# davide-coccomini/MINTIME-Multi-Identity-size-iNvariant-TIMEsformer-for-Video-Deepfake-Detection

Measured on AMD Instinct MI355X. Metric: clips/sec (8-frame, 2-identity, 224^2 crops) fwd+bwd, higher is better.
Workload: dtype f32; 1 GPU; config 3: EfficientNet-B0 + SizeInvariantTimeSformer(dim 512, depth 9, heads 8), B=32/GPU, 8 frames, 2 identities (identity-masked), 224x224 crops, random-init seeded weights (restored before every step), train-mode BN + drop-connect 0.2, step = fwd + BCE loss + bwd + SGD(lr .01, wd 1e-4); global_batch=32, frames=8, parallelism=dp1

## Files before the change

mintime-multi-identity-size-invariant-timesformer-for-video-deepfake-detection_amd/csrc/gemm_planes.hip:

```cpp
#include "../../include/mintime_hip.h"
#include "common.hpp"
#include "gemm_planes_launch.hpp"
#include "gemm_geometry.hpp"
#include "det.hpp"
#include <string.h>

using namespace mt;

namespace {

__device__ __forceinline__ void to_blk_block(const float* __restrict__ src, int64_t ld, int R, int C, const PlaneRef& o, int rb, int cb, int lane) {
  const int r = rb * 32 + (lane >> 1), c = cb * 16 + (lane & 1) * 8;
  float x[8] = {0.f, 0.f, 0.f, 0.f, 0.f, 0.f, 0.f, 0.f};
  if (r < R) {
    const float* s = src + (int64_t)r * ld + c;
    if (c + 8 <= C && ((ld & 3) == 0) && (((uintptr_t)src & 15) == 0)) {
      const float4 u = *reinterpret_cast<const float4*>(s), v = *reinterpret_cast<const float4*>(s + 4);
      x[0] = u.x; x[1] = u.y; x[2] = u.z; x[3] = u.w; x[4] = v.x; x[5] = v.y; x[6] = v.z; x[7] = v.w;
    } else {
#pragma unroll
      for (int e = 0; e < 8; ++e) if (c + e < C) x[e] = s[e];
    }
  }
  planes_store8(o, r, c, x);
}

__global__ __launch_bounds__(256) void split_planes_blk_kernel(const float* __restrict__ src, int64_t ld, int R, int C, PlaneRef o) {
  const int wave = threadIdx.x >> 6, lane = threadIdx.x & 63;
  const int rb = blockIdx.y, cb = blockIdx.x * 4 + wave;
  if (cb >= o.cb16) return;
  to_blk_block(src, ld, R, C, o, rb, cb, lane);
}

__global__ __launch_bounds__(256) void bn_bwd_apply_planes_kernel(const float* __restrict__ du, const float* __restrict__ z,
                                                                  const float* __restrict__ kabc, int R, int C, PlaneRef o) {
  const int wave = threadIdx.x >> 6, lane = threadIdx.x & 63;
  const int rb = blockIdx.y, cb = blockIdx.x * 4 + wave;
  if (cb >= o.cb16) return;
  const int r = rb * 32 + (lane >> 1), c = cb * 16 + (lane & 1) * 8;
  float x[8] = {0.f, 0.f, 0.f, 0.f, 0.f, 0.f, 0.f, 0.f};
  if (r < R) {
#pragma unroll
    for (int e = 0; e < 8; e += 4) {
      if (c + e + 4 <= C) {
        const float4 a = *reinterpret_cast<const float4*>(du + (int64_t)r * C + c + e), b = *reinterpret_cast<const float4*>(z + (int64_t)r * C + c + e);
        const float4 ka = *reinterpret_cast<const float4*>(kabc + c + e), kb = *reinterpret_cast<const float4*>(kabc + C + c + e),
                     kc = *reinterpret_cast<const float4*>(kabc + 2 * C + c + e);
        x[e] = fmaf(ka.x, a.x, fmaf(kb.x, b.x, kc.x)); x[e + 1] = fmaf(ka.y, a.y, fmaf(kb.y, b.y, kc.y));
        x[e + 2] = fmaf(ka.z, a.z, fmaf(kb.z, b.z, kc.z)); x[e + 3] = fmaf(ka.w, a.w, fmaf(kb.w, b.w, kc.w));
      }
    }
  }
  planes_store8(o, r, c, x);
}

struct SplitItem { const float* src; __bf16* planes; int64_t rows, cols, first; };

__global__ __launch_bounds__(256) void split_planes_blk_multi_kernel(const SplitItem* __restrict__ items, int count, int64_t total) {
  const int64_t wb = (int64_t)blockIdx.x * 4 + (threadIdx.x >> 6);
  if (wb >= total) return;
  int lo = 0, hi = count - 1;
  while (lo < hi) { const int mid = (lo + hi + 1) >> 1; if (items[mid].first <= wb) lo = mid; else hi = mid - 1; }
  const SplitItem it = items[lo];
  const int R = (int)it.rows, Cc = (int)it.cols;
  const int cb16 = (Cc + 15) >> 4, rp = (R + 31) & ~31;
  const int64_t loc = wb - it.first;
  const PlaneRef o{it.planes, (int64_t)rp * cb16 * 16, cb16, rp};
  to_blk_block(it.src, Cc, R, Cc, o, (int)(loc / cb16), (int)(loc % cb16), threadIdx.x & 63);
}

constexpr int kSkMaxGrid = 1024;
constexpr int64_t kSkFlagBytes = 4096;

int cu_count() {
  static int cus[64] = {0};
  int dev = 0;
  (void)hipGetDevice(&dev);
  int& c = cus[dev & 63];
  if (c == 0) {
    hipDeviceProp_t pr;
    c = hipGetDeviceProperties(&pr, dev) == hipSuccess && pr.multiProcessorCount > 0 ? pr.multiProcessorCount : 256;
  }
  return c;
}

int g_persist = -1;
int persist_blocks() {
  if (g_persist < 0) {
    g_persist = env_int("MT_PLANES_PERSIST", 0);
    if (g_persist < 0 || g_persist > 4) g_persist = 0;
  }
  return g_persist;
}

}

extern "C" int mt_gemm_planes_set_persist(int blocks_per_cu) {
  const int prev = persist_blocks();
  g_persist = blocks_per_cu < 0 || blocks_per_cu > 4 ? 0 : blocks_per_cu;
  return prev;
}

extern "C" int64_t mt_gemm_planes_workspace_bytes(void) { return kSkFlagBytes + (int64_t)kSkMaxGrid * 128 * 128 * 4; }

extern "C" int64_t mt_planes_elems(int rows, int cols) {
  if (rows <= 0 || cols <= 0) return 0;
  return (int64_t)((rows + 31) & ~31) * ((cols + 15) & ~15);
}

extern "C" int mt_split_planes_blk(const float* src, int64_t ld, int rows, int cols, void* planes, void* stream) {
  if (!src || !planes) return fail(MT_ERR_ARG, "mt_split_planes_blk: null pointer");
  if (rows <= 0 || cols <= 0 || ld < cols) return fail(MT_ERR_ARG, "mt_split_planes_blk: bad shape %d x %d (ld %lld)", rows, cols, (long long)ld);
  if ((uintptr_t)planes & 15) return fail(MT_ERR_ARG, "mt_split_planes_blk: planes must be 16-byte aligned");
  const int cb16 = (cols + 15) >> 4, rp = (rows + 31) & ~31;
  const PlaneRef o{reinterpret_cast<__bf16*>(planes), (int64_t)rp * cb16 * 16, cb16, rp};
  hipLaunchKernelGGL(split_planes_blk_kernel, dim3((cb16 + 3) / 4, rp / 32), dim3(256), 0, (hipStream_t)stream, src, ld, rows, cols, o);
  return check_launch("mt_split_planes_blk");
}

extern "C" int mt_bn_bwd_apply_planes(const float* du, const float* z, const float* kabc, void* planes, int rows, int C, void* stream) {
  if (!du || !z || !kabc || !planes || rows <= 0 || C <= 0) return fail(MT_ERR_ARG, "mt_bn_bwd_apply_planes: bad arguments");
  if ((C & 3) || (((uintptr_t)du | (uintptr_t)z | (uintptr_t)kabc | (uintptr_t)planes) & 15))
    return fail(MT_ERR_ARG, "mt_bn_bwd_apply_planes: C %% 4 == 0 and 16-byte alignment");
  const int cb16 = (C + 15) >> 4, rp = (rows + 31) & ~31;
  const PlaneRef o{reinterpret_cast<__bf16*>(planes), (int64_t)rp * cb16 * 16, cb16, rp};
  hipLaunchKernelGGL(bn_bwd_apply_planes_kernel, dim3((cb16 + 3) / 4, rp / 32), dim3(256), 0, (hipStream_t)stream, du, z, kabc, rows, C, o);
  return check_launch("mt_bn_bwd_apply_planes");
}

extern "C" int mt_split_planes_blk_multi(const void* items, int count, int64_t total_blocks, void* stream) {
  if (!items || count <= 0 || total_blocks <= 0) return fail(MT_ERR_ARG, "mt_split_planes_blk_multi: bad arguments");
  hipLaunchKernelGGL(split_planes_blk_multi_kernel, dim3((unsigned)((total_blocks + 3) / 4)), dim3(256), 0, (hipStream_t)stream,
                     reinterpret_cast<const SplitItem*>(items), count, total_blocks);
  return check_launch("mt_split_planes_blk_multi");
}

static int gemm_planes_impl(const mt_gemm_planes_desc* d, void* stream) {
  if (!d || !d->a_planes || !d->b_planes) return fail(MT_ERR_ARG, "mt_gemm_planes: null operand planes");
  if (d->M <= 0 || d->N <= 0 || d->K <= 0) return fail(MT_ERR_ARG, "mt_gemm_planes: bad shape %d %d %d", d->M, d->N, d->K);
  if (((uintptr_t)d->a_planes & 15) || ((uintptr_t)d->b_planes & 15) || ((uintptr_t)d->c_planes & 15))
    return fail(MT_ERR_ARG, "mt_gemm_planes: planes must be 16-byte aligned");
  const int op = d->op, epi = d->epilogue;
  const bool cpl = d->c_planes != nullptr;
  if (!d->C && !cpl) return fail(MT_ERR_ARG, "mt_gemm_planes: no output");
  if (cpl && epi != MT_EPI_GEGLU && epi != MT_EPI_GEGLU_BWD) return fail(MT_ERR_UNSUPPORTED, "mt_gemm_planes: plane output only from the GEGLU pair");
  if (epi == MT_EPI_BIAS_RES && !d->R) return fail(MT_ERR_ARG, "mt_gemm_planes: BIAS_RES needs R");
  if (epi == MT_EPI_GEGLU && (d->n_half * 2 != d->N || (d->n_half & 63))) return fail(MT_ERR_ARG, "mt_gemm_planes GEGLU: N must be 2*n_half, n_half %% 64 == 0");
  if (epi == MT_EPI_GEGLU_BWD && (!d->C2 || d->n_half != d->N || (d->n_half & 31)))
    return fail(MT_ERR_ARG, "mt_gemm_planes GEGLU_BWD: needs C2, n_half == N and n_half %% 32 == 0");
  hipStream_t s = (hipStream_t)stream;
  const bool high = matmul_precision() == MT_PRECISION_HIGH;
  const int np = high ? 2 : 3;
  auto launch = [&](int skm, const GemmArgs& ga, dim3 g) {
    return high ? launch_planes_high(op, epi, cpl, skm, ga, g, s) : launch_planes_form<3>(op, epi, cpl, skm, ga, g, s);
  };

  const int a_rows = op == MT_OP_TN ? d->K : d->M, a_cols = op == MT_OP_TN ? d->M : d->K;
  const int b_rows = op == MT_OP_NT ? d->N : d->K, b_cols = op == MT_OP_NT ? d->K : d->N;
  GemmArgs a;
  memset(&a, 0, sizeof(a));
  a.C = d->C; a.M = d->M; a.N = d->N; a.K = d->K; a.ldc = d->ldc;
  a.a_planes = d->a_planes; a.a_pstride = mt_planes_elems(a_rows, a_cols); a.lda = (a_cols + 15) >> 4;
  a.b_planes = d->b_planes; a.b_pstride = mt_planes_elems(b_rows, b_cols); a.ldb = (b_cols + 15) >> 4;
  if (6 * a.a_pstride > 0xFFFFFFFFll || 6 * a.b_pstride > 0xFFFFFFFFll)
    return fail(MT_ERR_UNSUPPORTED, "mt_gemm_planes: an operand's planes span %lld bytes (> 4 GB: 32-bit DMA offsets); use mt_gemm for it (lib.planes_fit)",
                (long long)(6 * (a.a_pstride > a.b_pstride ? a.a_pstride : a.b_pstride)));
  a.bias = d->bias; a.R = d->R; a.ldr = d->ldr; a.C2 = d->C2; a.ldc2 = d->ldc2; a.n_half = d->n_half; a.col_sum = d->col_sum;
  a.hw = 1; a.stats_slots = d->stats_slots != 0 ? d->stats_slots : 1; a.stats = d->stats; a.b_hw = 1; a.e_hw = 1;
  if (epi == MT_EPI_STATS && !d->stats) return fail(MT_ERR_ARG, "mt_gemm_planes: STATS needs stats");
  if (epi == MT_EPI_GEGLU_BWD)
    if (int rc = det_gemm_colsum_setup(a.det, d->M, d->n_half, d->col_sum, s)) return rc;
  if (cpl) {
    const int c_cols = epi == MT_EPI_GEGLU ? d->n_half : 2 * d->n_half;
    a.c_planes = d->c_planes; a.c_pstride = mt_planes_elems(d->M, c_cols); a.ldcp = (c_cols + 15) >> 4;
  }

  const TileGrid tg = tile_grid(d->M, d->N, 128, 128, (int64_t)128 * d->K * 2 * np);
  const int m_tiles = tg.m_tiles, n_tiles = tg.n_tiles;
  if (op == MT_OP_TN) {
    if (epi != MT_EPI_ATOMIC) return fail(MT_ERR_UNSUPPORTED, "mt_gemm_planes TN: ATOMIC epilogue only (C pre-zeroed)");
    static const int target = env_int("MT_WGRAD_BLOCKS", 640);
    const SplitK sk = split_k_ranges(d->K, m_tiles * n_tiles, d->split_k, target, 16, K_XCD);
    a.k_chunk = sk.k_chunk; a.xcd_k = sk.xcd_k;
    if (int rc = det_gemm_setup(a.C, a.ldc, a.det_slab, d->M, d->N, sk.ranges, false, s)) return rc;
    return launch(0, a, dim3(m_tiles * n_tiles, sk.grid_y, 1));
  }
  dim3 grid(tg.grid_x, 1, 1);
  a.group_n = tg.group_n;
  static const int prio = env_int("MT_PLANES_MAIN_PRIO", 0);
  a.wave_prio = prio;
  bool sk = false;
  if (d->sk_workspace && d->sk_workspace_bytes >= mt_gemm_planes_workspace_bytes() && !((uintptr_t)d->sk_workspace & 255)) {
    int g = cu_count() * 2 / 8 * 8;
    if (g > kSkMaxGrid) g = kSkMaxGrid;
    const int64_t units = (int64_t)m_tiles * n_tiles * (((d->K + 15) / 16 + 1) / 2);
    if (g >= 8 && units >= (int64_t)g * 2 && units < (1ll << 30)) {
      sk = true;
      grid = dim3((unsigned)g, 1, 1);
      a.sk_on = 1;
      a.sk_flags = reinterpret_cast<int*>(d->sk_workspace);
      a.sk_ws = reinterpret_cast<float*>(reinterpret_cast<char*>(d->sk_workspace) + kSkFlagBytes);
    }
  }
  if (!sk && !cpl && (epi == MT_EPI_STORE || epi == MT_EPI_BIAS_RES)) {
    const int per_cu = persist_blocks();
    const int g = cu_count() * per_cu / 8 * 8;
    if (per_cu > 0 && g >= 8 && m_tiles * n_tiles > g) {
      const dim3 pg((unsigned)g, 1, 1);
      const bool nt_store = op == MT_OP_NT && epi == MT_EPI_STORE, nt_bias_res = op == MT_OP_NT && epi == MT_EPI_BIAS_RES;
      const bool nn_store = op == MT_OP_NN && epi == MT_EPI_STORE;
      if (nt_store || nt_bias_res || nn_store) return launch(2, a, pg);
    }
  }
  return launch(sk ? 1 : 0, a, grid);
}

extern "C" int mt_gemm_planes(const mt_gemm_planes_desc* d, void* stream) {
  const int rc = gemm_planes_impl(d, stream);
  if (rc) { (void)mt::det_gemm_finish(nullptr, false); return rc; }
  return mt::det_gemm_finish((hipStream_t)stream, true);
}
```

mintime-multi-identity-size-invariant-timesformer-for-video-deepfake-detection_amd/csrc/gemm_planes.hpp:

```cpp
#pragma once
#include "gemm_split.hpp"
#include "planes.hpp"

#ifndef MT_PLANES_ABLATE
#define MT_PLANES_ABLATE 0
#endif
#ifndef MT_PLANES_EPI_ABLATE
#define MT_PLANES_EPI_ABLATE 0
#endif
#ifndef MT_PLANES_PRIO
#define MT_PLANES_PRIO 0
#endif

namespace mt {

typedef short s16x4_t __attribute__((ext_vector_type(4)));
enum : int { BAL_NONE = 0, BAL_PAIR = 1, BAL_PHASE = 2 };

__device__ __forceinline__ void lds_dma16_s(const void* sbase, unsigned voff, unsigned lds_byte_addr) {
  unsigned keep;
  asm volatile("s_mov_b32 %0, m0\n\ts_mov_b32 m0, %3\n\ts_nop 0\n\tglobal_load_lds_dwordx4 %1, %2\n\ts_mov_b32 m0, %0"
               : "=&s"(keep) : "v"(voff), "s"(sbase), "s"(lds_byte_addr) : "memory");
}

__device__ __forceinline__ void planes_emit_tile(const float (&v)[16], float* wl, const PlaneRef& o, int row0, int col0, int M, int lane) {
  const int col_l = lane & 31, row_h = (lane >> 5) * 4;
#pragma unroll
  for (int r = 0; r < 16; ++r) wl[((r & 3) + 8 * (r >> 2) + row_h) * 36 + col_l] = v[r];
  asm volatile("s_waitcnt lgkmcnt(0)" ::: "memory");
#pragma unroll
  for (int pass = 0; pass < 2; ++pass) {
    const int g = pass * 64 + lane, row = g >> 2, cg = g & 3;
    const float4 lo = *reinterpret_cast<const float4*>(wl + row * 36 + cg * 8);
    const float4 hi = *reinterpret_cast<const float4*>(wl + row * 36 + cg * 8 + 4);
    const int rg = row0 + row, cgl = col0 + cg * 8;
    const bool live = rg < M;
    const float x[8] = {live ? lo.x : 0.f, live ? lo.y : 0.f, live ? lo.z : 0.f, live ? lo.w : 0.f,
                        live ? hi.x : 0.f, live ? hi.y : 0.f, live ? hi.z : 0.f, live ? hi.w : 0.f};
    if (rg < o.rows_pad && cgl < o.cb16 * 16) { if (MT_PLANES_EPI_ABLATE & 8) { if (x[0] + x[7] == 123.456f) o.p[0] = (__bf16)1.f; } else planes_store8(o, rg, cgl, x); }
  }
  asm volatile("s_waitcnt lgkmcnt(0)" ::: "memory");
}

template <int TM, int TN, int EPI>
__device__ __forceinline__ void planes_epilogue(const GemmArgs& p, f32x16 (&acc)[TM][TN], int m0, int n0, int wm, int wn, int lane, float* wl) {
  static_assert(EPI == EPI_GEGLU || EPI == EPI_GEGLU_BWD, "plane output: the GEGLU pair");
  const PlaneRef o{reinterpret_cast<__bf16*>(p.c_planes), p.c_pstride, (int)p.ldcp, (p.M + 31) & ~31};
  const int col_l = lane & 31, row_h = (lane >> 5) * 4;
  const int mw = m0 + wm * TM * 32;
  if constexpr (EPI == EPI_GEGLU) {
    const int j = (n0 >> 1) + wn * 32 + col_l;
    const bool jok = j < p.n_half;
    const float ba = (jok && p.bias) ? p.bias[j] : 0.f;
    const float bg = (jok && p.bias) ? p.bias[p.n_half + j] : 0.f;
#pragma unroll
    for (int i = 0; i < TM; ++i) {
      float hv[16];
#pragma unroll
      for (int r = 0; r < 16; ++r) {
        const int m = mw + i * 32 + row_h + (r & 3) + 8 * (r >> 2);
        const float a = acc[i][0][r] + ba, g = acc[i][1][r] + bg;
        hv[r] = a * gelu_erf(g);
        if (m < p.M && jok) {
          if (p.C2) *reinterpret_cast<float2*>(p.C2 + (int64_t)m * p.ldc2 + 2 * j) = make_float2(a, g);
          if (p.C) p.C[(int64_t)m * p.ldc + j] = hv[r];
        }
      }
      planes_emit_tile(hv, wl, o, mw + i * 32, (n0 >> 1) + wn * 32, p.M, lane);
    }
  } else {
    f32x16 dgs[TM][TN];
    float s1[TN], s2[TN];
#pragma unroll
    for (int j = 0; j < TN; ++j) {
      const int n = n0 + wn * TN * 32 + j * 32 + col_l;
      const bool nok = n < p.N;
      s1[j] = 0.f; s2[j] = 0.f;
#pragma unroll
      for (int i = 0; i < TM; ++i) {
        float2 ag[16];
#pragma unroll
        for (int r = 0; r < 16; ++r) {
          const int m = mw + i * 32 + row_h + (r & 3) + 8 * (r >> 2);
          ag[r] = ((MT_PLANES_EPI_ABLATE & 1) || !(m < p.M && nok)) ? make_float2(0.3f, 0.1f)
                                                                     : *reinterpret_cast<const float2*>(p.C2 + (int64_t)m * p.ldc2 + 2 * n);
        }
#pragma unroll
        for (int r = 0; r < 16; ++r) {
          const int m = mw + i * 32 + row_h + (r & 3) + 8 * (r >> 2);
          const float v = acc[i][j][r];
          float gl, gr;
          if (MT_PLANES_EPI_ABLATE & 2) { gl = ag[r].y; gr = ag[r].y + 1.f; } else gelu_erf_both(ag[r].y, gl, gr);
          const bool live = m < p.M && nok;
          const float da = live ? v * gl : 0.f, dg = live ? v * ag[r].x * gr : 0.f;
          acc[i][j][r] = da;
          dgs[i][j][r] = dg;
          s1[j] += da; s2[j] += dg;
        }
        __builtin_amdgcn_sched_barrier(0);
      }
    }
#pragma unroll
    for (int j = 0; j < TN; ++j) {
      const int n = n0 + wn * TN * 32 + j * 32 + col_l;
      const bool nok = n < p.N;
#pragma unroll
      for (int i = 0; i < TM; ++i) {
        float da[16], dg[16];
#pragma unroll
        for (int r = 0; r < 16; ++r) {
          da[r] = acc[i][j][r]; dg[r] = dgs[i][j][r];
          const int m = mw + i * 32 + row_h + (r & 3) + 8 * (r >> 2);
          if (p.C && m < p.M && nok) { p.C[(int64_t)m * p.ldc + n] = da[r]; p.C[(int64_t)m * p.ldc + p.n_half + n] = dg[r]; }
        }
        if (MT_PLANES_EPI_ABLATE & 4) { if (da[3] + dg[5] == 123.456f) p.col_sum[0] = 1.f; }
        else if (n0 + wn * TN * 32 + j * 32 < p.N) {
          planes_emit_tile(da, wl, o, mw + i * 32, n0 + wn * TN * 32 + j * 32, p.M, lane);
          planes_emit_tile(dg, wl, o, mw + i * 32, p.n_half + n0 + wn * TN * 32 + j * 32, p.M, lane);
        }
      }
      if (p.col_sum && !(MT_PLANES_EPI_ABLATE & 16)) {
        float t1 = s1[j], t2 = s2[j];
        t1 += __shfl_xor(t1, 32);
        t2 += __shfl_xor(t2, 32);
        if (lane < 32 && nok) {
          if (p.det.vals) {
            const int rk = mw >> 5;
            det_put(p.det, n >> 5, rk, n & 31, t1);
            det_put(p.det, (p.n_half + n) >> 5, rk, n & 31, t2);
            if (rk == 0 && (n & 31) == 0) { det_base(p.det, n >> 5, n); det_base(p.det, (p.n_half + n) >> 5, p.n_half + n); }
          } else {
            atomicAdd(p.col_sum + n, t1);
            atomicAdd(p.col_sum + p.n_half + n, t2);
          }
        }
      }
    }
  }
}

template <int BM, int BN>
__device__ __forceinline__ void sk_tile_coords(const GemmArgs& p, int t, int& mt_, int& nt_) {
  const int n_tiles = (p.N + BN - 1) / BN, m_tiles = (p.M + BM - 1) / BM;
  if (p.group_n > 0) {
    const int q = m_tiles >> 3, r = m_tiles & 7;
    int xcd = 0, base = 0;
    for (; xcd < 7; ++xcd) {
      const int cnt = (q + (xcd < r ? 1 : 0)) * n_tiles;
      if (t < base + cnt) break;
      base += cnt;
    }
    const int rows = q + (xcd < r ? 1 : 0);
    const int row0 = xcd < r ? xcd * (q + 1) : r * (q + 1) + (xcd - r) * q;
    const int idx = t - base;
    const int per_group = rows * p.group_n;
    const int g = idx / per_group;
    const int rem = idx - g * per_group;
    const int groups = (n_tiles + p.group_n - 1) / p.group_n;
    const int gw = (g == groups - 1) ? n_tiles - g * p.group_n : p.group_n;
    const int ml = rem / gw;
    mt_ = row0 + ml;
    nt_ = g * p.group_n + (rem - ml * gw);
  } else {
    mt_ = t / n_tiles;
    nt_ = t - mt_ * n_tiles;
  }
}

template <int WAVES_M, int WAVES_N, int TM, int TN, bool AKM, bool BKM, int EPI, int STAGES, int MINW, int BAL, bool CPL = false, int SKM = 0, int NP = 3>
__global__ __launch_bounds__(WAVES_M * WAVES_N * 64, MINW)
void gemm_planes_kernel(const GemmArgs p) {
  constexpr int NW = WAVES_M * WAVES_N;
  constexpr int BM = WAVES_M * TM * 32;
  constexpr int BN = WAVES_N * TN * 32;
  constexpr int BK = 16;
  constexpr int A_PLANE = BM * 32, B_PLANE = BN * 32;
  static_assert(NP == 2 || NP == 3, "two or three pieces per operand");
  constexpr int STAGE = NP * (A_PLANE + B_PLANE);
  constexpr int PPA = A_PLANE / 1024, PPB = B_PLANE / 1024;
  constexpr int PA = NP * PPA, PB = NP * PPB;
  static_assert((PA + PB) % NW == 0, "every wavefront must issue the same number of DMA pieces");
  constexpr int IPW = (PA + PB) / NW;
  static_assert(STAGES >= 2 && STAGES <= 4, "2..4 stages");
  static_assert((!AKM || BM == 128) && (!BKM || BN == 128), "k-major images are laid out for 128-column tiles");
  constexpr bool SK = SKM == 1, PS = SKM == 2;
  static_assert(!SK || !AKM, "stream-K: forward / data-gradient forms (weight gradients split K over the grid already)");
  static_assert(!PS || (!AKM && !CPL && STAGES == 2 && EPI != EPI_GEGLU && BAL != BAL_PHASE), "persistent form: NT / NN, fp32 output, ring of two");
  constexpr bool PAIR = BAL == BAL_PAIR, PHASE = BAL == BAL_PHASE;

  extern __shared__ __attribute__((aligned(16))) unsigned char smem_pl[];
  const unsigned lds_base = (unsigned)(uintptr_t)(__attribute__((address_space(3))) unsigned char*)smem_pl;

  const int tid = threadIdx.x;
  const int lane = tid & 63;
  const int wave = __builtin_amdgcn_readfirstlane(tid >> 6);
  const int wm = wave / WAVES_N;
  const int wn = wave % WAVES_N;

  const __bf16* a_base = reinterpret_cast<const __bf16*>(p.a_planes);
  const __bf16* b_base = reinterpret_cast<const __bf16*>(p.b_planes);

  int a_frag[TM], b_frag[TN];
  {
    const int kh = lane >> 5;
    const int g = lane >> 4, i16 = lane & 15;
    const int ktr = 8 * (g >> 1) + (i16 >> 2);
    const int swz = 2 * (i16 >> 2);
#pragma unroll
    for (int i = 0; i < TM; ++i) {
      if constexpr (!AKM) {
        const int row = wm * TM * 32 + i * 32 + (lane & 31);
        a_frag[i] = row * 32 + ((kh ^ ((row >> 3) & 1)) << 4);
      } else {
        const int seg = (wm * TM * 32 + i * 32) / 16 + (g & 1);
        a_frag[i] = ktr * 256 + ((seg ^ swz) * 32) + (i16 & 3) * 8;
      }
    }
#pragma unroll
    for (int j = 0; j < TN; ++j) {
      if constexpr (!BKM) {
        const int row = wn * TN * 32 + j * 32 + (lane & 31);
        b_frag[j] = row * 32 + ((kh ^ ((row >> 3) & 1)) << 4);
      } else {
        const int seg = (wn * TN * 32 + j * 32) / 16 + (g & 1);
        b_frag[j] = ktr * 256 + ((seg ^ swz) * 32) + (i16 & 3) * 8;
      }
    }
  }

  struct Frags { bf16x8_t a0[TM], a1[TM], a2[NP == 3 ? TM : 1], b0[TN], b1[TN], b2[NP == 3 ? TN : 1]; };
  typedef __attribute__((address_space(3))) s16x4_t* lds_tr_p;
  typedef __attribute__((address_space(3))) const unsigned char* lds_cp;
  auto tr_read = [&](const unsigned char* base) -> bf16x8_t {
    lds_cp a = (lds_cp)base;
    const s16x4_t lo = __builtin_amdgcn_ds_read_tr16_b64_v4i16((lds_tr_p)a);
    const s16x4_t hi = __builtin_amdgcn_ds_read_tr16_b64_v4i16((lds_tr_p)(a + 1024));
    union { s16x4_t h[2]; bf16x8_t v; } u;
    u.h[0] = lo; u.h[1] = hi;
    return u.v;
  };

  auto read_frags = [&](int slot, Frags& f) {
    const unsigned char* sa = smem_pl + slot * STAGE;
    const unsigned char* sb = sa + NP * A_PLANE;
    if (MT_PLANES_ABLATE & 4) {
#pragma unroll
      for (int e = 0; e < 8; ++e) {
#pragma unroll
        for (int i = 0; i < TM; ++i) { f.a0[i][e] = (__bf16)(float)(lane + e + i); f.a1[i][e] = (__bf16)(float)(lane - e); if constexpr (NP == 3) f.a2[i][e] = (__bf16)(float)(lane ^ e); }
#pragma unroll
        for (int j = 0; j < TN; ++j) { f.b0[j][e] = (__bf16)(float)(lane * 2 + e + j); f.b1[j][e] = (__bf16)(float)(lane + 3 * e); if constexpr (NP == 3) f.b2[j][e] = (__bf16)(float)(3 + e); }
      }
      return;
    }
#pragma unroll
    for (int i = 0; i < TM; ++i) {
      if constexpr (!AKM) {
        f.a0[i] = *reinterpret_cast<const bf16x8_t*>(sa + a_frag[i]);
        f.a1[i] = *reinterpret_cast<const bf16x8_t*>(sa + A_PLANE + a_frag[i]);
        if constexpr (NP == 3) f.a2[i] = *reinterpret_cast<const bf16x8_t*>(sa + 2 * A_PLANE + a_frag[i]);
      } else {
        f.a0[i] = tr_read(sa + a_frag[i]);
        f.a1[i] = tr_read(sa + A_PLANE + a_frag[i]);
        if constexpr (NP == 3) f.a2[i] = tr_read(sa + 2 * A_PLANE + a_frag[i]);
      }
    }
#pragma unroll
    for (int j = 0; j < TN; ++j) {
      if constexpr (!BKM) {
        f.b0[j] = *reinterpret_cast<const bf16x8_t*>(sb + b_frag[j]);
        f.b1[j] = *reinterpret_cast<const bf16x8_t*>(sb + B_PLANE + b_frag[j]);
        if constexpr (NP == 3) f.b2[j] = *reinterpret_cast<const bf16x8_t*>(sb + 2 * B_PLANE + b_frag[j]);
      } else {
        f.b0[j] = tr_read(sb + b_frag[j]);
        f.b1[j] = tr_read(sb + B_PLANE + b_frag[j]);
        if constexpr (NP == 3) f.b2[j] = tr_read(sb + 2 * B_PLANE + b_frag[j]);
      }
    }
  };

  auto negate = [&](bf16x8_t& v, unsigned mask) {
    uint4 u = *reinterpret_cast<uint4*>(&v);
    u.x ^= mask; u.y ^= mask; u.z ^= mask; u.w ^= mask;
    v = *reinterpret_cast<bf16x8_t*>(&u);
  };

  f32x16 acc[TM][TN];
  f32x16 nacc[PAIR ? TM : 1][PAIR ? TN : 1];

  auto mma = [&](Frags& f, auto odd_c, unsigned phase_mask) {
    constexpr bool ODD = PAIR && decltype(odd_c)::value;
    if (MT_PLANES_ABLATE & 16) {
      float z = 0.f;
#pragma unroll
      for (int i = 0; i < TM; ++i) { z += (float)f.a0[i][0] + (float)f.a1[i][1]; if constexpr (NP == 3) z += (float)f.a2[i][2]; }
#pragma unroll
      for (int j = 0; j < TN; ++j) { z += (float)f.b0[j][0] + (float)f.b1[j][1]; if constexpr (NP == 3) z += (float)f.b2[j][2]; }
      acc[0][0][0] += z;
      return;
    }
#define MT_TERM(X, Y)                                                                                        \
  _Pragma("unroll") for (int i = 0; i < TM; ++i) _Pragma("unroll") for (int j = 0; j < TN; ++j)                 \
      acc[i][j] = __builtin_amdgcn_mfma_f32_32x32x16_bf16(f.X[i], f.Y[j], acc[i][j], 0, 0, 0);
#define MT_NTERM(X, Y)                                                                                       \
  _Pragma("unroll") for (int i = 0; i < TM; ++i) _Pragma("unroll") for (int j = 0; j < TN; ++j)                 \
      nacc[i][j] = __builtin_amdgcn_mfma_f32_32x32x16_bf16(f.X[i], f.Y[j], nacc[i][j], 0, 0, 0);
    if constexpr (PHASE) {
#pragma unroll
      for (int i = 0; i < TM; ++i) { negate(f.a0[i], phase_mask); negate(f.a1[i], phase_mask); if constexpr (NP == 3) negate(f.a2[i], phase_mask); }
    }
    if constexpr (ODD) {
#pragma unroll
      for (int i = 0; i < TM; ++i) negate(f.a0[i], 0x80008000u);
      if constexpr (NP == 3) { MT_TERM(a2, b0) MT_TERM(a1, b1) MT_NTERM(a0, b2) }
      MT_TERM(a1, b0) MT_NTERM(a0, b1) MT_NTERM(a0, b0)
    } else {
      if constexpr (NP == 3) { MT_TERM(a2, b0) MT_TERM(a1, b1) MT_TERM(a0, b2) }
      MT_TERM(a1, b0) MT_TERM(a0, b1) MT_TERM(a0, b0)
    }
#undef MT_TERM
#undef MT_NTERM
  };
  auto flip_acc = [&]() {
#pragma unroll
    for (int i = 0; i < TM; ++i)
#pragma unroll
      for (int j = 0; j < TN; ++j)
#pragma unroll
        for (int r = 0; r < 16; ++r) acc[i][j][r] = -acc[i][j][r];
  };
#define MT_PL_BARRIER() do { if (!(MT_PLANES_ABLATE & 2)) __builtin_amdgcn_s_barrier(); } while (0)

  auto run_piece = [&](int mt_, int nt_, int k_begin, int kt_lo, int nk) {
    const int m0 = mt_ * BM, n0 = nt_ * BN;
    unsigned voff[IPW];
    bool is_a[IPW];
#pragma unroll
    for (int j = 0; j < IPW; ++j) {
      const int q = wave * IPW + j;
      is_a[j] = q < PA;
      const int qq = is_a[j] ? q : q - PA;
      const int plane = is_a[j] ? qq / PPA : qq / PPB;
      const int piece = is_a[j] ? qq % PPA : qq % PPB;
      const int64_t pstride = is_a[j] ? p.a_pstride : p.b_pstride;
      const int64_t cb16 = is_a[j] ? p.lda : p.ldb;
      const bool kmaj = is_a[j] ? AKM : BKM;
      int64_t off;
      if (!kmaj) {
        const int row = lane >> 1, slot = lane & 1;
        const int kh = slot ^ ((row >> 3) & 1);
        int g0;
        int lim;
        if (is_a[j]) { g0 = m0 + piece * 32; lim = p.M; }
        else if constexpr (EPI == EPI_GEGLU) {
          static_assert(EPI != EPI_GEGLU || TN == 2, "GEGLU wants TN == 2");
          const int w = piece >> 1, sel = piece & 1;
          g0 = sel * p.n_half + (n0 >> 1) + w * 32; lim = 2 * p.n_half;
          if ((n0 >> 1) + w * 32 >= p.n_half) g0 = 0;
        } else { g0 = n0 + piece * 32; lim = p.N; }
        if (g0 >= lim) g0 = (lim - 1) & ~31;
        off = plane * pstride + (int64_t)(g0 >> 5) * cb16 * 512 + row * 16 + kh * 8;
      } else {
        const int kl = piece * 4 + (lane >> 4), s16 = lane & 15;
        const int seg = (s16 >> 1) ^ (2 * (kl & 3)), half = s16 & 1;
        int cb = ((is_a[j] ? m0 : n0) >> 4) + seg;
        const int cbmax = (int)cb16 - 1;
        cb = cb < cbmax ? cb : cbmax;
        off = plane * pstride + (int64_t)cb * 512 + kl * 16 + half * 8;
      }
      voff[j] = (unsigned)(off * 2);
    }

    auto issue = [&](int kt, int slot) {
      if (MT_PLANES_ABLATE & 1) return;
      const int kb = k_begin + (kt_lo + kt) * BK;
      const __bf16* as = a_base + (AKM ? ((int64_t)(kb >> 5) * p.lda * 512 + (kb & 31) * 16) : (int64_t)(kb >> 4) * 512);
      const __bf16* bs = b_base + (BKM ? ((int64_t)(kb >> 5) * p.ldb * 512 + (kb & 31) * 16) : (int64_t)(kb >> 4) * 512);
      const unsigned dst = lds_base + (unsigned)(slot * STAGE);
#pragma unroll
      for (int j = 0; j < IPW; ++j)
        lds_dma16_s(is_a[j] ? as : bs, voff[j], dst + (unsigned)((wave * IPW + j) * 1024));
    };

#pragma unroll
    for (int i = 0; i < TM; ++i)
#pragma unroll
      for (int j = 0; j < TN; ++j)
#pragma unroll
        for (int r = 0; r < 16; ++r) { acc[i][j][r] = 0.f; if constexpr (PAIR) nacc[i][j][r] = 0.f; }

    const int q1 = PHASE ? nk >> 2 : nk, q2 = PHASE ? nk - (nk >> 2) : nk;

#pragma unroll
    for (int s = 0; s < STAGES - 1; ++s)
      if (s < nk) issue(s, s);
    int slot = 0;
    auto step = [&](int kt, auto odd_c) {
      const int later = min(STAGES - 2, nk - 1 - kt);
      if (later >= 2) wait_vmcnt<2 * IPW>();
      else if (later == 1) wait_vmcnt<IPW>();
      else wait_vmcnt<0>();
      MT_PL_BARRIER();
      int nslot = slot + STAGES - 1; nslot = nslot >= STAGES ? nslot - STAGES : nslot;
      if (kt + STAGES - 1 < nk) issue(kt + STAGES - 1, nslot);
      Frags f;
      read_frags(slot, f);
      unsigned mask = 0;
      if constexpr (PHASE) {
        if (kt == q1 || kt == q2) flip_acc();
        mask = (kt >= q1 && kt < q2) ? 0x80008000u : 0u;
      }
      mma(f, odd_c, mask);
      slot = slot + 1 >= STAGES ? 0 : slot + 1;
    };
    for (int kt = 0; kt < nk; kt += 2) {
      step(kt, std::false_type{});
      if (kt + 1 >= nk) break;
      step(kt + 1, std::true_type{});
    }
    if constexpr (PHASE) {
      if (q2 >= nk && q1 < nk) flip_acc();
    }
    if constexpr (PAIR) {
#pragma unroll
      for (int i = 0; i < TM; ++i)
#pragma unroll
        for (int j = 0; j < TN; ++j)
#pragma unroll
          for (int r = 0; r < 16; ++r) acc[i][j][r] -= nacc[i][j][r];
#pragma unroll
      for (int i = 0; i < TM; ++i)
#pragma unroll
        for (int j = 0; j < TN; ++j) asm volatile("" : "+v"(acc[i][j]));
    }
  };

  auto epilogue = [&](int mt_, int nt_, int split_idx = -1) {
    if (MT_PLANES_ABLATE & 8) {
      float sacc = 0.f;
#pragma unroll
      for (int i = 0; i < TM; ++i)
#pragma unroll
        for (int j = 0; j < TN; ++j)
#pragma unroll
          for (int r = 0; r < 16; ++r) sacc += acc[i][j][r];
      if (sacc == 123.456f) p.C[0] = sacc;
      return;
    }
    int m0e = mt_ * BM, n0e = nt_ * BN, lane_e = lane;
    asm volatile("" : "+s"(m0e), "+s"(n0e), "+v"(lane_e));
    if constexpr (CPL) {
      static_assert(!CPL || STAGES * STAGE >= NW * 32 * 36 * 4, "the plane epilogue's LDS patches live in the main loop's stages");
      __syncthreads();
      planes_epilogue<TM, TN, EPI>(p, acc, m0e, n0e, wm, wn, lane_e, reinterpret_cast<float*>(smem_pl) + wave * (32 * 36));
    } else {
      gemm_epilogue<TM, TN, EPI>(p, acc, m0e, n0e, wm, wn, lane_e, split_idx);
    }
  };

  if (p.wave_prio == 1) __builtin_amdgcn_s_setprio(1);
  else if (p.wave_prio == 2) __builtin_amdgcn_s_setprio(2);
  else if (p.wave_prio == 3) __builtin_amdgcn_s_setprio(3);
  if (MT_PLANES_PRIO == 1) {
    const unsigned hwid = __builtin_amdgcn_s_getreg((4 << 0) | (0 << 6) | (3 << 11));
    if (__builtin_amdgcn_readfirstlane(hwid) & 1) __builtin_amdgcn_s_setprio(1);
  } else if (MT_PLANES_PRIO == 2) {
    if ((blockIdx.x >> 8) & 1) __builtin_amdgcn_s_setprio(1);
  }

  if constexpr (PS) {
    const int Q = gridDim.x >> 3, xcd = blockIdx.x & 7, q = blockIdx.x >> 3;
    const int n_tiles = (p.N + BN - 1) / BN, m_tiles = (p.M + BM - 1) / BM;
    int base = 0, cnt;
    if (p.group_n > 0) {
      const int qq = m_tiles >> 3, rr = m_tiles & 7;
      for (int i = 0; i < xcd; ++i) base += (qq + (i < rr ? 1 : 0)) * n_tiles;
      cnt = (qq + (xcd < rr ? 1 : 0)) * n_tiles;
    } else {
      const int T = m_tiles * n_tiles, per = T >> 3, rem = T & 7;
      base = xcd * per + min(xcd, rem);
      cnt = per + (xcd < rem ? 1 : 0);
    }
    if (q >= cnt) return;
    const int nk = (p.K + BK - 1) / BK;
    bool is_a[IPW];
    int pl_[IPW], pc_[IPW];
#pragma unroll
    for (int j = 0; j < IPW; ++j) {
      const int qj = wave * IPW + j;
      is_a[j] = qj < PA;
      const int qx = is_a[j] ? qj : qj - PA;
      pl_[j] = is_a[j] ? qx / PPA : qx / PPB;
      pc_[j] = is_a[j] ? qx % PPA : qx % PPB;
    }
    auto setup = [&](int mt_, int nt_, unsigned (&voff)[IPW]) {
      const int m0 = mt_ * BM, n0 = nt_ * BN;
#pragma unroll
      for (int j = 0; j < IPW; ++j) {
        const int64_t pstride = is_a[j] ? p.a_pstride : p.b_pstride;
        const int64_t cb16 = is_a[j] ? p.lda : p.ldb;
        const bool kmaj = is_a[j] ? AKM : BKM;
        int64_t off;
        if (!kmaj) {
          const int row = lane >> 1, sl = lane & 1;
          const int kh = sl ^ ((row >> 3) & 1);
          int g0 = (is_a[j] ? m0 : n0) + pc_[j] * 32;
          const int lim = is_a[j] ? p.M : p.N;
          if (g0 >= lim) g0 = (lim - 1) & ~31;
          off = pl_[j] * pstride + (int64_t)(g0 >> 5) * cb16 * 512 + row * 16 + kh * 8;
        } else {
          const int kl = pc_[j] * 4 + (lane >> 4), s16 = lane & 15;
          const int seg = (s16 >> 1) ^ (2 * (kl & 3)), half = s16 & 1;
          int cb = ((is_a[j] ? m0 : n0) >> 4) + seg;
          const int cbmax = (int)cb16 - 1;
          cb = cb < cbmax ? cb : cbmax;
          off = pl_[j] * pstride + (int64_t)cb * 512 + kl * 16 + half * 8;
        }
        voff[j] = (unsigned)(off * 2);
      }
    };
    auto issue = [&](const unsigned (&voff)[IPW], int kt, int slot_) {
      if (MT_PLANES_ABLATE & 1) return;
      const int kb = kt * BK;
      const __bf16* as = a_base + (AKM ? ((int64_t)(kb >> 5) * p.lda * 512 + (kb & 31) * 16) : (int64_t)(kb >> 4) * 512);
      const __bf16* bs = b_base + (BKM ? ((int64_t)(kb >> 5) * p.ldb * 512 + (kb & 31) * 16) : (int64_t)(kb >> 4) * 512);
      const unsigned dst = lds_base + (unsigned)(slot_ * STAGE);
#pragma unroll
      for (int j = 0; j < IPW; ++j) lds_dma16_s(is_a[j] ? as : bs, voff[j], dst + (unsigned)((wave * IPW + j) * 1024));
    };
    int i = q, mt_, nt_;
    sk_tile_coords<BM, BN>(p, base + i, mt_, nt_);
    unsigned vc[IPW], vn[IPW];
    setup(mt_, nt_, vc);
    issue(vc, 0, 0);
    int slot = 0;
    while (true) {
      const int inext = i + Q;
      const bool has_next = inext < cnt;
      int mtn = 0, ntn = 0;
      if (has_next) {
        sk_tile_coords<BM, BN>(p, base + inext, mtn, ntn);
        setup(mtn, ntn, vn);
      }
#pragma unroll
      for (int ii = 0; ii < TM; ++ii)
#pragma unroll
        for (int jj = 0; jj < TN; ++jj)
#pragma unroll
          for (int r = 0; r < 16; ++r) { acc[ii][jj][r] = 0.f; if constexpr (PAIR) nacc[ii][jj][r] = 0.f; }
      auto step = [&](int kt, auto odd_c) {
        wait_vmcnt<0>();
        MT_PL_BARRIER();
        const int nslot = slot ^ 1;
        if (kt + 1 < nk) issue(vc, kt + 1, nslot);
        else if (has_next) issue(vn, 0, nslot);
        Frags f;
        read_frags(slot, f);
        mma(f, odd_c, 0u);
        slot = nslot;
      };
      for (int kt = 0; kt < nk; kt += 2) {
        step(kt, std::false_type{});
        if (kt + 1 >= nk) break;
        step(kt + 1, std::true_type{});
      }
      if constexpr (PAIR) {
#pragma unroll
        for (int ii = 0; ii < TM; ++ii)
#pragma unroll
          for (int jj = 0; jj < TN; ++jj)
#pragma unroll
            for (int r = 0; r < 16; ++r) acc[ii][jj][r] -= nacc[ii][jj][r];
#pragma unroll
        for (int ii = 0; ii < TM; ++ii)
#pragma unroll
          for (int jj = 0; jj < TN; ++jj) asm volatile("" : "+v"(acc[ii][jj]));
      }
      epilogue(mt_, nt_);
      if (!has_next) break;
      i = inext; mt_ = mtn; nt_ = ntn;
#pragma unroll
      for (int j = 0; j < IPW; ++j) vc[j] = vn[j];
    }
  } else if constexpr (!SK) {
    int mt_, nt_;
    int k_begin = 0, k_end = p.K;
    int split_idx = blockIdx.y;
    if (p.xcd_k) {
      const int tiles = gridDim.x, lin = blockIdx.y * gridDim.x + blockIdx.x;
      const int xcd = lin & 7, idx = lin >> 3;
      const int split = xcd + 8 * (idx / tiles), t = idx % tiles;
      const int n_tiles = (p.N + BN - 1) / BN, m_tiles = (p.M + BM - 1) / BM;
      if (m_tiles >= n_tiles) { mt_ = t / n_tiles; nt_ = t - mt_ * n_tiles; }
      else { nt_ = t / m_tiles; mt_ = t - nt_ * m_tiles; }
      k_begin = split * p.k_chunk;
      k_end = min(p.K, k_begin + p.k_chunk);
      if (k_begin >= k_end) return;
      split_idx = split;
    } else {
      if (!tile_coords<BM, BN>(p, mt_, nt_)) return;
      if (p.k_chunk > 0) {
        k_begin = blockIdx.y * p.k_chunk;
        k_end = min(p.K, k_begin + p.k_chunk);
        if (k_begin >= k_end) return;
      }
    }
    const int nk = (k_end - k_begin + BK - 1) / BK;
    if (nk <= 0) return;
    run_piece(mt_, nt_, k_begin, 0, nk);
    epilogue(mt_, nt_, split_idx);
  } else {
    const int G = gridDim.x;
    const int L = (blockIdx.x & 7) * (G >> 3) + (blockIdx.x >> 3);
    const int nkt = (p.K + BK - 1) / BK;
    const int npt = (nkt + 1) >> 1;
    const int U = ((p.N + BN - 1) / BN) * ((p.M + BM - 1) / BM) * npt;
    const int uq = U / G, ur = U % G;
    int u = L * uq + min(L, ur);
    const int u_end = u + uq + (L < ur ? 1 : 0);
    constexpr int SLAB = BM * BN;
    while (u < u_end) {
      const int t = u / npt;
      const int kt0 = 2 * (u - t * npt);
      const int ulen = min(npt - (u - t * npt), u_end - u);
      const int len = min(nkt - kt0, 2 * ulen);
      int mt_, nt_;
      sk_tile_coords<BM, BN>(p, t, mt_, nt_);
      __builtin_amdgcn_s_barrier();
      run_piece(mt_, nt_, 0, kt0, len);
      u += ulen;
      if (len != nkt) {
        int lane_s = lane, wave_s = wave;
        asm volatile("" : "+v"(lane_s), "+s"(wave_s));
        const int my_off = wave_s * (TM * TN * 1024) + lane_s * 4;
        if (kt0 != 0) {
          float* slab = p.sk_ws + (int64_t)L * SLAB + my_off;
#pragma unroll
          for (int i = 0; i < TM; ++i)
#pragma unroll
            for (int j = 0; j < TN; ++j)
#pragma unroll
              for (int q = 0; q < 4; ++q)
                *reinterpret_cast<float4*>(slab + ((i * TN + j) * 4 + q) * 256) =
                    make_float4(acc[i][j][4 * q], acc[i][j][4 * q + 1], acc[i][j][4 * q + 2], acc[i][j][4 * q + 3]);
          asm volatile("s_waitcnt vmcnt(0)" ::: "memory");
          __syncthreads();
          if (tid == 0) {
            __builtin_amdgcn_fence(__ATOMIC_RELEASE, "agent");
            asm volatile("s_waitcnt vmcnt(0)" ::: "memory");
            __hip_atomic_store(p.sk_flags + L, 1, __ATOMIC_RELAXED, __HIP_MEMORY_SCOPE_AGENT);
          }
          continue;
        }
        int covered = ulen;
        for (int lb = L + 1; covered < npt; ++lb) {
          const int span = uq + (lb < ur ? 1 : 0);
          if (tid == 0) {
            int spins = 0;
            while (__hip_atomic_load(p.sk_flags + lb, __ATOMIC_RELAXED, __HIP_MEMORY_SCOPE_AGENT) == 0) {
              __builtin_amdgcn_s_sleep(8);
              if (++spins > (1 << 24)) break;
            }
            __builtin_amdgcn_fence(__ATOMIC_ACQUIRE, "agent");
          }
          __syncthreads();
          const float* slab = p.sk_ws + (int64_t)lb * SLAB + my_off;
#pragma unroll
          for (int i = 0; i < TM; ++i)
#pragma unroll
            for (int j = 0; j < TN; ++j)
#pragma unroll
              for (int q = 0; q < 4; ++q) {
                const float4 v = *reinterpret_cast<const float4*>(slab + ((i * TN + j) * 4 + q) * 256);
                acc[i][j][4 * q] += v.x; acc[i][j][4 * q + 1] += v.y; acc[i][j][4 * q + 2] += v.z; acc[i][j][4 * q + 3] += v.w;
              }
          asm volatile("s_waitcnt vmcnt(0)" ::: "memory");
          __syncthreads();
          if (tid == 0) __hip_atomic_store(p.sk_flags + lb, 0, __ATOMIC_RELAXED, __HIP_MEMORY_SCOPE_AGENT);
          covered += min(npt - covered, span);
        }
      }
      epilogue(mt_, nt_);
    }
  }
#undef MT_PL_BARRIER
}

}
```

Baseline: 719.0 clips/s.

## Restructure GEGLU backward epilogue with buffer loads and per-column-block software pipelining

The GEGLU backward epilogue now reads the saved (a, g) pairs through a bounds-checked raw buffer resource, so out-of-range lanes get zeros without per-element predication. It also prefetches the next column block's pairs while the current block is written out. The full dgs[TM][TN] register array becomes a per-j dgj[TM] buffer and each column block is stored right after it is computed, which should lower register pressure and overlap loads with stores. The column-sum reduction moves after the loop. A new ldc2 range check keeps the 32-bit buffer offsets valid, and the ag[TM][16] prefetch array costs registers in exchange.

```diff
diff --git a/mintime-multi-identity-size-invariant-timesformer-for-video-deepfake-detection_amd/csrc/gemm_planes.hip b/mintime-multi-identity-size-invariant-timesformer-for-video-deepfake-detection_amd/csrc/gemm_planes.hip
--- a/mintime-multi-identity-size-invariant-timesformer-for-video-deepfake-detection_amd/csrc/gemm_planes.hip
+++ b/mintime-multi-identity-size-invariant-timesformer-for-video-deepfake-detection_amd/csrc/gemm_planes.hip
@@ -148,6 +148,8 @@
   if (epi == MT_EPI_GEGLU && (d->n_half * 2 != d->N || (d->n_half & 63))) return fail(MT_ERR_ARG, "mt_gemm_planes GEGLU: N must be 2*n_half, n_half %% 64 == 0");
   if (epi == MT_EPI_GEGLU_BWD && (!d->C2 || d->n_half != d->N || (d->n_half & 31)))
     return fail(MT_ERR_ARG, "mt_gemm_planes GEGLU_BWD: needs C2, n_half == N and n_half %% 32 == 0");
+  if (epi == MT_EPI_GEGLU_BWD && cpl && (d->ldc2 < 2 * (int64_t)d->n_half || d->ldc2 >= (1ll << 24)))
+    return fail(MT_ERR_ARG, "mt_gemm_planes GEGLU_BWD: ldc2 %lld must hold 2*n_half columns and stay below 2^24", (long long)d->ldc2);
   hipStream_t s = (hipStream_t)stream;
   const bool high = matmul_precision() == MT_PRECISION_HIGH;
   const int np = high ? 2 : 3;
diff --git a/mintime-multi-identity-size-invariant-timesformer-for-video-deepfake-detection_amd/csrc/gemm_planes.hpp b/mintime-multi-identity-size-invariant-timesformer-for-video-deepfake-detection_amd/csrc/gemm_planes.hpp
--- a/mintime-multi-identity-size-invariant-timesformer-for-video-deepfake-detection_amd/csrc/gemm_planes.hpp
+++ b/mintime-multi-identity-size-invariant-timesformer-for-video-deepfake-detection_amd/csrc/gemm_planes.hpp
@@ -24,6 +24,7 @@
 }
 
 __device__ __forceinline__ void planes_emit_tile(const float (&v)[16], float* wl, const PlaneRef& o, int row0, int col0, int M, int lane) {
+  asm volatile("" : "+v"(lane));
   const int col_l = lane & 31, row_h = (lane >> 5) * 4;
 #pragma unroll
   for (int r = 0; r < 16; ++r) wl[((r & 3) + 8 * (r >> 2) + row_h) * 36 + col_l] = v[r];
@@ -69,49 +70,62 @@
       planes_emit_tile(hv, wl, o, mw + i * 32, (n0 >> 1) + wn * 32, p.M, lane);
     }
   } else {
-    f32x16 dgs[TM][TN];
+    const int nu0 = n0 + wn * TN * 32;
+    const int64_t u_left = ((int64_t)(p.M - 1 - mw) * p.ldc2 + 2 * (p.N - nu0)) * 4;
+    const unsigned u_bytes = (mw < p.M && nu0 < p.N) ? (unsigned)(u_left < 0xFFFFFFFFll ? u_left : 0xFFFFFFFFll) : 0u;
+    const __amdgpu_buffer_rsrc_t u_rsrc = __builtin_amdgcn_make_buffer_rsrc(
+        const_cast<float*>(p.C2) + (int64_t)mw * p.ldc2 + 2 * nu0, 0, (int)u_bytes, 0x00020000);
+    const unsigned u_lane = (unsigned)((row_h * p.ldc2 + 2 * col_l) * 4);
+    float2 ag[TM][16];
+    auto load_half = [&](int j) {
+#pragma unroll
+      for (int i = 0; i < TM; ++i)
+#pragma unroll
+        for (int r = 0; r < 16; ++r) {
+          const unsigned u_row = (unsigned)(((i * 32 + (r & 3) + 8 * (r >> 2)) * p.ldc2 + 2 * j * 32) * 4);
+          typedef unsigned u32x2_t __attribute__((ext_vector_type(2)));
+          const u32x2_t w = __builtin_amdgcn_raw_buffer_load_b64(u_rsrc, u_lane + u_row, 0, 0);
+          ag[i][r] = (MT_PLANES_EPI_ABLATE & 1) ? make_float2(0.3f, 0.1f) : make_float2(__uint_as_float(w.x), __uint_as_float(w.y));
+        }
+    };
     float s1[TN], s2[TN];
+    load_half(0);
 #pragma unroll
     for (int j = 0; j < TN; ++j) {
       const int n = n0 + wn * TN * 32 + j * 32 + col_l;
       const bool nok = n < p.N;
+      f32x16 dgj[TM];
       s1[j] = 0.f; s2[j] = 0.f;
 #pragma unroll
       for (int i = 0; i < TM; ++i) {
-        float2 ag[16];
-#pragma unroll
-        for (int r = 0; r < 16; ++r) {
-          const int m = mw + i * 32 + row_h + (r & 3) + 8 * (r >> 2);
-          ag[r] = ((MT_PLANES_EPI_ABLATE & 1) || !(m < p.M && nok)) ? make_float2(0.3f, 0.1f)
-                                                                     : *reinterpret_cast<const float2*>(p.C2 + (int64_t)m * p.ldc2 + 2 * n);
-        }
 #pragma unroll
         for (int r = 0; r < 16; ++r) {
           const int m = mw + i * 32 + row_h + (r & 3) + 8 * (r >> 2);
           const float v = acc[i][j][r];
           float gl, gr;
-          if (MT_PLANES_EPI_ABLATE & 2) { gl = ag[r].y; gr = ag[r].y + 1.f; } else gelu_erf_both(ag[r].y, gl, gr);
+          if (MT_PLANES_EPI_ABLATE & 2) { gl = ag[i][r].y; gr = ag[i][r].y + 1.f; } else gelu_erf_both(ag[i][r].y, gl, gr);
           const bool live = m < p.M && nok;
-          const float da = live ? v * gl : 0.f, dg = live ? v * ag[r].x * gr : 0.f;
+          float da = live ? v * gl : 0.f, dg = live ? v * ag[i][r].x * gr : 0.f;
+          asm volatile("" : "+v"(da), "+v"(dg));
           acc[i][j][r] = da;
-          dgs[i][j][r] = dg;
+          dgj[i][r] = dg;
           s1[j] += da; s2[j] += dg;
-        }
-        __builtin_amdgcn_sched_barrier(0);
-      }
-    }
-#pragma unroll
-    for (int j = 0; j < TN; ++j) {
-      const int n = n0 + wn * TN * 32 + j * 32 + col_l;
-      const bool nok = n < p.N;
+          if ((r & 3) == 3) __builtin_amdgcn_sched_barrier(0);
+        }
+      }
+      if (j + 1 < TN) load_half(j + 1);
+      __builtin_amdgcn_sched_barrier(0);
 #pragma unroll
       for (int i = 0; i < TM; ++i) {
         float da[16], dg[16];
 #pragma unroll
-        for (int r = 0; r < 16; ++r) {
-          da[r] = acc[i][j][r]; dg[r] = dgs[i][j][r];
-          const int m = mw + i * 32 + row_h + (r & 3) + 8 * (r >> 2);
-          if (p.C && m < p.M && nok) { p.C[(int64_t)m * p.ldc + n] = da[r]; p.C[(int64_t)m * p.ldc + p.n_half + n] = dg[r]; }
+        for (int r = 0; r < 16; ++r) { da[r] = acc[i][j][r]; dg[r] = dgj[i][r]; }
+        if (p.C) {
+#pragma unroll
+          for (int r = 0; r < 16; ++r) {
+            const int m = mw + i * 32 + row_h + (r & 3) + 8 * (r >> 2);
+            if (m < p.M && nok) { p.C[(int64_t)m * p.ldc + n] = da[r]; p.C[(int64_t)m * p.ldc + p.n_half + n] = dg[r]; }
+          }
         }
         if (MT_PLANES_EPI_ABLATE & 4) { if (da[3] + dg[5] == 123.456f) p.col_sum[0] = 1.f; }
         else if (n0 + wn * TN * 32 + j * 32 < p.N) {
@@ -119,11 +133,15 @@
           planes_emit_tile(dg, wl, o, mw + i * 32, p.n_half + n0 + wn * TN * 32 + j * 32, p.M, lane);
         }
       }
-      if (p.col_sum && !(MT_PLANES_EPI_ABLATE & 16)) {
+    }
+    if (p.col_sum && !(MT_PLANES_EPI_ABLATE & 16)) {
+#pragma unroll
+      for (int j = 0; j < TN; ++j) {
+        const int n = n0 + wn * TN * 32 + j * 32 + col_l;
         float t1 = s1[j], t2 = s2[j];
         t1 += __shfl_xor(t1, 32);
         t2 += __shfl_xor(t2, 32);
-        if (lane < 32 && nok) {
+        if (lane < 32 && n < p.N) {
           if (p.det.vals) {
             const int rk = mw >> 5;
             det_put(p.det, n >> 5, rk, n & 31, t1);
```

Measured after the change: 724.0 clips/s (median of 6 runs). No clear change (+0.7%).
